# ndming/GS-2M

Measured on AMD Instinct MI355X. Metric: train views/s (fwd+bwd raster) at 1M Gaussians 1080p, higher is better.
Workload: dtype f32; 1 GPU; BASELINE configs[2] (c3): 1000000 synthetic Gaussians (SH deg 3), 1 camera 1920x1080 per GPU, feature_count=9, fwd+bwd at the op boundary; gaussians=1000000, visible=844909, num_rendered=2709460, width=1920, height=1080, feature_count=9, parallelism=view-parallel x1, views_per_rank=1

## Files before the change

gs-2m_amd/csrc/api.hip:

```cpp
#include "common.h"
#include <atomic>
#include <mutex>
#include <chrono>
#include <dlfcn.h>

#define HIP_TRY(expr)                          \
    do {                                       \
        hipError_t e_ = (expr);                \
        if (e_ != hipSuccess) return GS2M_ERR_HIP; \
    } while (0)

namespace {

uint32_t higher_msb(uint32_t n) {
    uint32_t msb = sizeof(n) * 4;
    uint32_t step = msb;
    while (step > 1) {
        step /= 2;
        if (n >> msb) msb += step; else msb -= step;
    }
    if (n >> msb) msb++;
    return msb;
}

// ... 6 lines not shown
};
LandRing g_land[64];
std::mutex g_land_mutex;
thread_local uint64_t t_last_token = 0;
thread_local long long t_rows_hint = -1;
thread_local long long t_units_hint = -1, t_units_from_token = -1;

static_assert(GS2M_NUM_STAGES == 10, "stage table");
enum Stage { ST_PREPROCESS = 0, ST_UNUSED1, ST_SCAN, ST_EMIT, ST_TILE_SORT, ST_LISTS, ST_BLEND_FWD, ST_UNUSED7,
             ST_BLEND_BWD, ST_GAUSSIAN_BWD, ST_COUNT };
constexpr int kMaxRecords = 8192;
struct Prof {
    std::atomic<int> mode{0};
    int n = 0;
    hipEvent_t ev[kMaxRecords][2];
    int stage[kMaxRecords];
    int created = 0;
    int every = 1;
    int seen3 = 0;
};
Prof g_prof;
std::mutex g_prof_mutex;
std::atomic<int> g_reference_binning{0};
std::atomic<int> g_spin_wait{1};
std::atomic<int> g_debug{0};
std::atomic<int> g_markers{0};

const char* const kStageNames[ST_COUNT] = {"preprocess", "-", "scan", "emit", "tile_sort", "depth_order+quad_lists", "blend_fwd", "-", "blend_bwd", "gaussian_bwd"};

struct Roctx {
    int (*push)(const char*) = nullptr;
    int (*pop)() = nullptr;
    bool tried = false;
    void load() {
        if (tried) return;
        tried = true;
        void* h = dlopen("libroctx64.so", RTLD_NOW | RTLD_GLOBAL);
        if (!h) h = dlopen("libroctx64.so.4", RTLD_NOW | RTLD_GLOBAL);
        if (!h) return;
        push = (int (*)(const char*))dlsym(h, "roctxRangePushA");
        pop = (int (*)())dlsym(h, "roctxRangePop");
    }
};
Roctx g_roctx;

struct StageTimer {
// ... 18 lines not shown
                (void)hipEventCreate(&g_prof.ev[slot][0]);
                (void)hipEventCreate(&g_prof.ev[slot][1]);
                g_prof.created = slot + 1;
            }
            g_prof.stage[slot] = stage;
        }
        (void)hipEventRecord(g_prof.ev[slot][0], s);
    }
    ~StageTimer() {
        if (slot >= 0) (void)hipEventRecord(g_prof.ev[slot][1], s);
        if (failed && g_debug.load(std::memory_order_relaxed) && *failed == 0) {
            hipError_t e = hipGetLastError();
            if (e == hipSuccess) e = hipStreamSynchronize(s);
            if (e != hipSuccess) *failed = stage + 1;
        }
        if (marked && g_roctx.pop) g_roctx.pop();
    }
};
#define DEBUG_CHECK()                                        \
    do {                                                     \
        if (failed_stage) return GS2M_ERR_STAGE(failed_stage - 1); \
    } while (0)

}

extern "C" {

char* gs2m_prealloc_alloc(size_t bytes, void* user) {
    gs2m_prealloc* p = static_cast<gs2m_prealloc*>(user);
    if (!p) return nullptr;
    p->requested = bytes;
    if (p->ptr && bytes <= p->capacity) return p->ptr;
    p->used_fallback = 1;
    return p->fallback ? p->fallback(bytes, p->fallback_user) : nullptr;
}

const char* gs2m_version(void) { return "gs2m_raster 0.5 (gfx950, round 5)"; }

static int forward_impl(gs2m_alloc_fn geometry_alloc, void* geometry_user, gs2m_alloc_fn binning_alloc,
                        void* binning_user, gs2m_alloc_fn image_alloc, void* image_user, int P, int D, int M,
                        const float* background, int width, int height, const float* means3D, const float* shs, const float* shs_rest,
                        const float* colors_precomp, const float* opacities, const float* scales, float scale_modifier,
                        const float* rotations, const float* cov3D_precomp, const float* features,
                        const float* viewmatrix, const float* projmatrix, const float* cam_pos, float tan_fovx,
                        float tan_fovy, int prefiltered, int feature_count, float* out_color, int* out_radii,
                        int* out_observe, float* out_buffer, void* stream_) {
// ... 262 lines not shown
    if (!sh_dc || !sh_rest) return GS2M_ERR_INVALID_ARG;
    return backward_impl(P, D, M, R, background, width, height, means3D, sh_dc, sh_rest, colors_precomp, scales, scale_modifier, rotations, cov3D_precomp, features, viewmatrix, projmatrix, campos, tan_fovx, tan_fovy, radii, buffer, geom_buffer, binning_buffer, image_buffer, feature_count, grad_colors, grad_buffer, dL_dmeans2D, dL_dconics, dL_dopacities, dL_dcolors, dL_dmeans3D, dL_dcov3D, dL_dsh_dc, dL_dsh_rest, dL_dscales, dL_drots, dL_dfeatures, scratch_alloc, scratch_user, stream_);
}

int gs2m_raster_mark_visible(int P, const float* means3D, const float* viewmatrix, const float* projmatrix,
                             uint8_t* present, void* stream_) {
    (void)projmatrix;
    if (P < 0) return GS2M_ERR_INVALID_ARG;
    if (P == 0) return GS2M_OK;
    if (!means3D || !viewmatrix || !present) return GS2M_ERR_INVALID_ARG;
    gs2m_launch_mark_visible(P, means3D, viewmatrix, present, (hipStream_t)stream_);
    HIP_TRY(hipGetLastError());
    return GS2M_OK;
}

int gs2m_set_reference_binning(int on) {
    g_reference_binning = on ? 1 : 0;
    return GS2M_OK;
}

int gs2m_set_tile_sort_policy(int policy) {
    if (policy < 0 || policy > 3) return GS2M_ERR_INVALID_ARG;
    gs2m_set_tile_sort_policy_impl(policy);
    return GS2M_OK;
}

int gs2m_set_debug(int on) {
    g_debug = on ? 1 : 0;
    return GS2M_OK;
}

int gs2m_set_markers(int on) {
    g_markers = on ? 1 : 0;
    if (on) {
        g_roctx.load();
        if (!g_roctx.push || !g_roctx.pop) return GS2M_ERR_UNSUPPORTED;
    }
    return GS2M_OK;
}

const char* gs2m_stage_name(int stage) { return stage >= 0 && stage < ST_COUNT ? kStageNames[stage] : "?"; }

int gs2m_set_spin_wait(int on) {
    g_spin_wait = on ? 1 : 0;
    return GS2M_OK;
}
// ... 119 lines not shown
```

gs-2m_amd/csrc/blend_bwd_q.hip:

```cpp
#include "common.h"

namespace {

typedef float v4f __attribute__((ext_vector_type(4)));
#ifdef GS2M_ROW_SECTORS
#define GS2M_ROW_ROUND(nv) ((((nv) + 7) / 8) * 8)
#else
#define GS2M_ROW_ROUND(nv) ((((nv) + 3) / 4) * 4)
#endif
typedef float v2f __attribute__((ext_vector_type(2)));
#ifndef GS2M_BWDQ_WAVES
#define GS2M_BWDQ_WAVES
#endif
#ifndef GS2M_BWDQ_UNROLL_B
#define GS2M_BWDQ_UNROLL_B 1
#endif

__device__ __forceinline__ void row_scan_affine2(float& Ax, float& Ay, float& Bx, float& By) {
#define GS2M_AFFINE_LEVEL(D)                                                             \
        "v_fmac_f32_dpp %2, %2, %0 row_shr:" #D " row_mask:0xf bank_mask:0xf\n\t"          \
        "v_fmac_f32_dpp %3, %3, %1 row_shr:" #D " row_mask:0xf bank_mask:0xf\n\t"          \
        "v_mul_f32_dpp %0, %0, %0 row_shr:" #D " row_mask:0xf bank_mask:0xf\n\t"           \
        "v_mul_f32_dpp %1, %1, %1 row_shr:" #D " row_mask:0xf bank_mask:0xf\n\t"
    asm("s_nop 1\n\t"
        GS2M_AFFINE_LEVEL(1)
        GS2M_AFFINE_LEVEL(2)
        GS2M_AFFINE_LEVEL(4)
        GS2M_AFFINE_LEVEL(8)
        : "+v"(Ax), "+v"(Ay), "+v"(Bx), "+v"(By));
#undef GS2M_AFFINE_LEVEL
}
__device__ __forceinline__ float row_shr1(float first, float v) {
    return __int_as_float(__builtin_amdgcn_update_dpp(__float_as_int(first), __float_as_int(v), 0x111 , 0xF, 0xF, false));
}

template <int FC>
__global__ void __launch_bounds__(64) GS2M_BWDQ_WAVES blend_bwd_q_kernel(
    const uint2* __restrict__ ranges, const uint2* __restrict__ qlist, const uint32_t* __restrict__ qlast,
    const uint32_t* __restrict__ qcount, const uint32_t* __restrict__ qrow,
    const float4* __restrict__ rec, int W, int H, int tiles_x, int tiles, const float* __restrict__ bg, int fc,
    const float* __restrict__ final_T,
    const uint32_t* __restrict__ n_contrib, const float* __restrict__ grad_color,
    const float* __restrict__ grad_buffer, float* __restrict__ rows) {
    constexpr int NV = ROW_FEAT + FC;
    constexpr int ROWF = GS2M_ROW_ROUND(NV);
    constexpr int RSTRIDE = ROWF;
    constexpr int NC = 3 + FC;
    constexpr int KK = (NC + 3) / 4;
#ifndef GS2M_BWDQ_GSTRIDE
#define GS2M_BWDQ_GSTRIDE 20
#endif
    constexpr int GST = GS2M_BWDQ_GSTRIDE;
    __shared__ __align__(16) float s_g[64][GST];
    __shared__ float2 s_T2[32];
    __shared__ float2 s_B2[32];
    __shared__ uint2 s_N2[32];
    __shared__ __align__(16) float s_out[16][ROWF];
    __shared__ uint32_t s_rowg[16];

    const int b = blockIdx.x;
    const int tile = (b >> 5) * 8 + (b & 7);
    const int quad = (b >> 3) & 3;
    if (tile >= tiles) return;
    const int lane = threadIdx.x;
    const int tile_x = tile % tiles_x, tile_y = tile / tiles_x;
    const int qx0 = tile_x * GS2M_TILE + (quad & 1) * 8, qy0 = tile_y * GS2M_TILE + (quad >> 1) * 8;
    if (qx0 >= W || qy0 >= H) return;
    const uint2 range = ranges[tile];

    uint32_t lastp;
    {
        const int px = qx0 + (lane & 7), py = qy0 + (lane >> 3);
        const bool inside = px < W && py < H;
        const size_t HW = (size_t)H * W, pix = (size_t)py * W + px;
        const float Tf = inside ? final_T[pix] : 0.f;
        lastp = inside ? n_contrib[pix] : 0u;
        float g[16];
#pragma unroll
        for (int k = 0; k < 16; k++) g[k] = 0.f;
        if (inside) {
            g[0] = grad_color[pix]; g[1] = grad_color[HW + pix]; g[2] = grad_color[2 * HW + pix];
#pragma unroll
            for (int ch = 0; ch < FC; ch++) g[3 + ch] = ch < fc ? grad_buffer[ch * HW + pix] : 0.f;
        }
#pragma unroll
        for (int q = 0; q < 4; q++)
            *reinterpret_cast<float4*>(&s_g[lane][4 * q]) = make_float4(g[4 * q], g[4 * q + 1], g[4 * q + 2], g[4 * q + 3]);
        const int pe = ((lane >> 3) * 4 + (lane & 3)) * 2 + ((lane >> 2) & 1);
        reinterpret_cast<float*>(s_T2)[pe] = Tf;
        reinterpret_cast<float*>(s_B2)[pe] = bg[0] * g[0] + bg[1] * g[1] + bg[2] * g[2];
        reinterpret_cast<uint32_t*>(s_N2)[pe] = lastp;
    }
    gs2m_sync();

    const int j = lane & 15, r = lane >> 4;
    const float qxr = (float)(qx0 + r), qyf = (float)qy0;
    const float halfW = 0.5f * W, halfH = 0.5f * H;

    float sx = 0.f, sy = 0.f, sA = 0.f, sB = 0.f, sC = 0.f, so = 0.f;
    float scB[KK];
#pragma unroll
    for (int k = 0; k < KK; k++) scB[k] = 0.f;
    const float* gA = &s_g[4 * (j & 3) + (j >> 2)][r];
    uint32_t spos = 0xFFFFFFFFu;
    const v2f pxf2 = {qxr, qxr + 4.0f};

    const uint32_t len = range.y - range.x;
    const uint2* list = qlist + (size_t)4 * range.x + (size_t)quad * len;
    const uint32_t* lrow = qrow + (size_t)4 * range.x + (size_t)quad * len;
    const int np = (int)qlast[tile * 4 + quad];
    const int ngroups = (np + 15) >> 4;
    struct Fill {
        float4 g0;
        float2 g1;
        float ch[KK];
        uint32_t pos1;
        uint32_t row;
    };
    struct Entry {
        uint2 e;
        uint32_t row;
    };
    auto load_entry = [&](int g) {
        const int p = np - 1 - (16 * g + j);
        Entry en;
        en.e = list[max(p, 0)];
        en.row = lrow[max(p, 0)];
        en.e.y = p >= 0 ? en.e.y + 1u : 0xFFFFFFFFu;
        return en;
    };
    auto load_fill = [&](const Entry en) {
        Fill f;
        const float4* p = rec + (size_t)(en.e.x & GS2M_GID_MASK) * REC_Q;
        f.g0 = p[REC_GEO0];
        f.g1 = *reinterpret_cast<const float2*>(p + REC_GEO1);
#pragma unroll
        for (int k = 0; k < KK; k++) f.ch[k] = reinterpret_cast<const float*>(p + REC_CH + k)[r];
        f.pos1 = en.e.y;
        f.row = en.row;
        return f;
    };
    auto row_ptr = [&](uint32_t row) -> float* {
        return reinterpret_cast<float*>(reinterpret_cast<float4*>(rows) + (size_t)(row * (uint32_t)(RSTRIDE / 4)));
    };
    Fill f;
    uint32_t row_cur = 0;
    Entry e_next = {make_uint2(0u, 0u), 0u};
    int g_cur = 0;
    auto issue_next = [&]() {
        if (g_cur + 1 < ngroups) f = load_fill(e_next);
        if (g_cur + 2 < ngroups) e_next = load_entry(g_cur + 2);
    };
    int pending = 0;
    auto flush_rows = [&]() {
        constexpr int RQ = ROWF / 4;
#pragma unroll
        for (int t0 = 0; t0 < 16 * RQ; t0 += GS2M_WAVE) {
            const int t = t0 + lane, e = t / RQ, q = t - e * RQ;
            if (t < 16 * RQ && e < pending)
                reinterpret_cast<float4*>(row_ptr(s_rowg[e]))[q] = *reinterpret_cast<const float4*>(&s_out[e][4 * q]);
        }
        pending = 0;
    };
    auto process_group = [&](int nvalid) {
        v4f acc1 = {0.f, 0.f, 0.f, 0.f};
        float U1 = 0.f, U2 = 0.f;
        v2f m0 = {0.f, 0.f}, m1 = {0.f, 0.f}, m2 = {0.f, 0.f};
        auto gc_block = [&](int b) {
            v4f a = {0.f, 0.f, 0.f, 0.f};
#pragma unroll
            for (int k = 0; k < KK; k++) a = __builtin_amdgcn_mfma_f32_16x16x4f32(gA[(16 * b) * GST + 4 * k], scB[k], a, 0, 0, 0);
            return a;
        };
        v4f gnext = gc_block(0);
// ... 82 lines not shown
            const auto x = __builtin_amdgcn_permlane32_swap(__float_as_uint(va), __float_as_uint(vb), false, false);
            const float hab = __uint_as_float(x[0]) + __uint_as_float(x[1]);
            const auto y = __builtin_amdgcn_permlane32_swap(__float_as_uint(vc), __float_as_uint(vd), false, false);
            const float hcd = __uint_as_float(y[0]) + __uint_as_float(y[1]);
            const auto z = __builtin_amdgcn_permlane16_swap(__float_as_uint(hab), __float_as_uint(hcd), false, false);
            return __uint_as_float(z[0]) + __uint_as_float(z[1]);
        };
        const v2f dxc = sx2 - pxf2;
        const float M0 = m0.x + m0.y, Sx = dxc.x * m0.x + dxc.y * m0.y, Sy = m1.x + m1.y;
        const float Sxx = (dxc.x * dxc.x) * m0.x + (dxc.y * dxc.y) * m0.y, Sxy = dxc.x * m1.x + dxc.y * m1.y, Syy = m2.x + m2.y;
        const float o0 = -halfW * (sA * Sx + sB * Sy), o1 = -halfH * (sC * Sy + sB * Sx), o2 = halfW * U1, o3 = halfH * U2;
        const float o7 = so > 0.f ? M0 * __builtin_amdgcn_rcpf(so) : 0.f;
        const float R1 = reduce4(o0, o2, o1, o3);
        const float R2 = reduce4(-0.5f * Sxx, -0.5f * Syy, -0.5f * Sxy, o7);
        s_out[j][r] = R1;
        s_out[j][4 + r] = R2;
        if (r == 0) s_rowg[j] = row_cur;
#pragma unroll
        for (int rr = 0; rr < 4; rr++)
            if (j < ROWF - ROW_COL) s_out[4 * r + rr][ROW_COL + j] = j < NC ? acc1[rr] : 0.f;
        pending = nvalid;
    };

    {
        const int n = (int)qcount[tile * 4 + quad];
        for (int i = np + lane; i < n; i += GS2M_WAVE) {
            float4* o4 = reinterpret_cast<float4*>(row_ptr(lrow[i]));
#pragma unroll
            for (int q4 = 0; q4 < ROWF / 4; q4++) o4[q4] = make_float4(0.f, 0.f, 0.f, 0.f);
        }
    }
    if (ngroups > 0) {
        f = load_fill(load_entry(0));
        e_next = load_entry(1);
        for (g_cur = 0; g_cur < ngroups; g_cur++) {
            sx = f.g0.x; sy = f.g0.y; sA = f.g0.z; sB = f.g0.w; sC = f.g1.x; so = f.g1.y;
#pragma unroll
            for (int k = 0; k < KK; k++) scB[k] = f.ch[k];
            spos = f.pos1;
            row_cur = f.row;
            process_group(min(16, np - 16 * g_cur));
        }
        asm volatile("s_waitcnt lgkmcnt(0)" ::: "memory");
        flush_rows();
    }
}

int fc_template(int fc) { return fc <= 1 ? 1 : (fc <= 5 ? 5 : (fc <= 9 ? 9 : 10)); }

}

int gs2m_row_floats(int fc) { return GS2M_ROW_ROUND(ROW_FEAT + fc_template(fc)); }

void gs2m_launch_blend_bwd_q(int W, int H, int tiles_x, int tiles_y, int fc, const float* bg, const GeomState& g,
                             const BinningState& b, const ImageState& im, const float* grad_color,
                             const float* grad_buffer, float* rows, hipStream_t s) {
    const int tiles = tiles_x * tiles_y;
    const int grid = ((tiles + 7) / 8) * 32;
#define GS2M_BWDQ(FC)                                                                                                      \
    blend_bwd_q_kernel<FC><<<grid, 64, 0, s>>>(im.ranges, b.qlist, im.qlast, im.qcount, b.qrow, g.rec, W, H, tiles_x, tiles, bg, fc, im.final_T, \
                                                  im.n_contrib, grad_color, grad_buffer, rows)
    switch (fc_template(fc)) {
        case 1: GS2M_BWDQ(1); break;
        case 5: GS2M_BWDQ(5); break;
        case 9: GS2M_BWDQ(9); break;
        default: GS2M_BWDQ(10); break;
    }
#undef GS2M_BWDQ
}
```

gs-2m_amd/csrc/blend_fwd_q.hip:

```cpp
#include "common.h"

namespace {

typedef float v2f __attribute__((ext_vector_type(2)));

template <int FC>
__global__ void __launch_bounds__(64) blend_fwd_q_kernel(
    const uint2* __restrict__ ranges, const uint2* __restrict__ qlist, const uint32_t* __restrict__ qcount,
    const float4* __restrict__ rec, int W, int H, int tiles_x, int tiles, const float* __restrict__ bg, int fc,
    float* __restrict__ out_color, float* __restrict__ out_buffer, float* __restrict__ final_T,
    uint32_t* __restrict__ n_contrib, int* __restrict__ observe, uint32_t* __restrict__ qlast) {
    constexpr int NC = 3 + FC;
    constexpr int KQ = (NC + 3) / 4;
    constexpr int NP = (NC + 1) / 2;

    const int b = blockIdx.x;
    const int tile = (b >> 5) * 8 + (b & 7);
    const int quad = (b >> 3) & 3;
    if (tile >= tiles) return;
    const int lane = threadIdx.x;
    const int tile_x = tile % tiles_x, tile_y = tile / tiles_x;
    const int qx0 = tile_x * GS2M_TILE + (quad & 1) * 8, qy0 = tile_y * GS2M_TILE + (quad >> 1) * 8;
    if (qx0 >= W || qy0 >= H) return;
    const int px = qx0 + (lane & 7), py = qy0 + (lane >> 3);
    const bool inside = px < W && py < H;
    const float pxf = (float)px, pyf = (float)py;

    const uint2 range = ranges[tile];
    const uint32_t len = range.y - range.x;
    const int n = __builtin_amdgcn_readfirstlane((int)qcount[tile * 4 + quad]);
    const uint2* list = qlist + (size_t)4 * range.x + (size_t)quad * len;

    constexpr int CH = 16;
    constexpr int NS = 2 + KQ;
    constexpr int BUFQ = NS * CH + CH / 2;
    __shared__ float4 s_buf[2 * BUFQ];
    uint32_t lds_zero;
    asm volatile("v_mov_b32 %0, 0" : "=v"(lds_zero));
    float4* const s_base = s_buf + lds_zero;
    auto q_at = [&](int buf, int slot, int jj) -> float4& { return s_base[buf * BUFQ + slot * CH + jj]; };
    auto e_at = [&](int buf, int jj) -> uint2& { return reinterpret_cast<uint2*>(s_base + buf * BUFQ + NS * CH)[jj]; };
    const int ej = lane & 15, eq = lane >> 4;
    auto quad_of = [](int slot) { return slot < 2 ? slot : slot + 1; };

    float T = 1.0f;
    uint32_t last_contributor = 0;
    v2f acc[NP];
#pragma unroll
    for (int k = 0; k < NP; k++) acc[k] = v2f{0.f, 0.f};
    typedef unsigned long long mask_t;
    mask_t live = __builtin_amdgcn_ballot_w64(inside);
    bool watch = true;
    int ilast = 0;

    auto eval = [&](const int i, const int buf, const int jj) {
        const float4 a = q_at(buf, 0, jj);
        const float2 b = *reinterpret_cast<const float2*>(&q_at(buf, 1, jj));
        float4 c[KQ];
#pragma unroll
        for (int q = 0; q < KQ; q++) c[q] = q_at(buf, 2 + q, jj);
        const uint2 ec = e_at(buf, jj);
        const float dx = a.x - pxf, dy = a.y - pyf;
        const float p2 = gs2m_power(dx, dy, a.z, a.w, b.x);
        const float alpha = fminf(0.99f, b.y * gs2m_exp(p2));
        const float test_T = T * (1.0f - alpha);
        const mask_t cand = live & __builtin_amdgcn_ballot_w64(p2 <= 0.0f) & __builtin_amdgcn_ballot_w64(alpha >= 1.0f / 255.0f);
        const mask_t fin = cand & __builtin_amdgcn_ballot_w64(test_T < 0.0001f);
        const mask_t contrib = cand & ~fin;
        live &= ~fin;
        if (contrib != 0ull) ilast = i + 1;
        float tw;
        asm("v_cndmask_b32_e64 %0, 0, %1, %2" : "=v"(tw) : "v"(T), "s"(contrib));
        const float w = alpha * tw;
        const v2f ww = {w, w};
#pragma unroll
        for (int q = 0; q < KQ; q++) {
            if (4 * q < NC) acc[2 * q] = __builtin_elementwise_fma(v2f{c[q].x, c[q].y}, ww, acc[2 * q]);
            if (4 * q + 2 < NC) acc[2 * q + 1] = __builtin_elementwise_fma(v2f{c[q].z, c[q].w}, ww, acc[2 * q + 1]);
        }
        const uint32_t pos1 = ec.y;
        asm("v_cndmask_b32_e64 %0, %0, %1, %2" : "+v"(last_contributor) : "v"(pos1), "s"(contrib));
        if (watch) {
            const mask_t half = contrib & __builtin_amdgcn_ballot_w64(T > 0.5f);
            if (half != 0ull) {
                if (lane == 0) atomicAdd(&observe[__builtin_amdgcn_readfirstlane(ec.x)], (int)__popcll(half));
            }
            watch = (live & __builtin_amdgcn_ballot_w64(T > 0.5f)) != 0ull;
        }
        asm("v_cndmask_b32_e64 %0, %0, %1, %2" : "+v"(T) : "v"(test_T), "s"(contrib));
        return live == 0ull;
    };

    const int nchunks = (n + CH - 1) / CH;
    auto load_entry = [&](int c) {
        return list[min(c * CH + ej, n - 1)];
    };
    struct Stage { float4 a, b; };
    auto load_quads = [&](const uint2 e) {
        Stage st;
        const float4* p = rec + (size_t)(e.x & GS2M_GID_MASK) * REC_Q;
        st.a = p[quad_of(eq)];
        st.b = eq + 4 < NS ? p[quad_of(eq + 4)] : make_float4(0.f, 0.f, 0.f, 0.f);
        return st;
    };
    auto park = [&](int buf, const uint2 e, const Stage& st) {
        q_at(buf, eq, ej) = st.a;
        if (eq + 4 < NS) q_at(buf, eq + 4, ej) = st.b;
        if (eq == 0) e_at(buf, ej) = make_uint2(e.x & GS2M_GID_MASK, e.y + 1u);
    };
    if (nchunks > 0) {
        uint2 e1 = load_entry(0);
        park(0, e1, load_quads(e1));
        e1 = nchunks > 1 ? load_entry(1) : e1;
        bool stop = false;
        for (int c = 0; c < nchunks && !stop; c++) {
            Stage st;
            const uint2 ecur = e1;
            if (c + 1 < nchunks) st = load_quads(ecur);
            if (c + 2 < nchunks) e1 = load_entry(c + 2);
            const int base = c * CH, buf = c & 1;
#pragma unroll
            for (int jj = 0; jj < CH; jj++) {
                if (base + jj >= n) break;
                if (eval(base + jj, buf, jj)) { stop = true; break; }
            }
            if (c + 1 < nchunks && !stop) park(buf ^ 1, ecur, st);
        }
    }

    if (lane == 0) qlast[tile * 4 + quad] = (uint32_t)ilast;
    if (inside) {
        const size_t HW = (size_t)H * W;
        const size_t pix = (size_t)py * W + px;
        final_T[pix] = T;
        n_contrib[pix] = last_contributor;
        out_color[pix] = acc[0][0] + T * bg[0];
        out_color[HW + pix] = acc[0][1] + T * bg[1];
        out_color[2 * HW + pix] = acc[1][0] + T * bg[2];
#pragma unroll
        for (int ch = 0; ch < GS2M_NUM_FEATURES; ch++) {
            const int cch = 3 + ch;
            out_buffer[ch * HW + pix] = (ch < FC && ch < fc) ? acc[(cch >> 1) < NP ? (cch >> 1) : 0][cch & 1] : 0.0f;
        }
    }
}

}

void gs2m_launch_blend_fwd_q(int W, int H, int tiles_x, int tiles_y, int fc, const float* bg, const GeomState& g,
                             const BinningState& b, const ImageState& im, float* out_color, float* out_buffer,
                             int* out_observe, hipStream_t s) {
    const int tiles = tiles_x * tiles_y;
    const int grid = ((tiles + 7) / 8) * 32;
    const int fct = fc <= 1 ? 1 : (fc <= 5 ? 5 : (fc <= 9 ? 9 : 10));
#define GS2M_FWDQ(FC)                                                                                                   \
    blend_fwd_q_kernel<FC><<<grid, 64, 0, s>>>(im.ranges, b.qlist, im.qcount, g.rec, W, H, tiles_x, tiles, bg, fc, out_color, \
                                               out_buffer, im.final_T, im.n_contrib, out_observe, im.qlast)
    switch (fct) {
        case 1: GS2M_FWDQ(1); break;
        case 5: GS2M_FWDQ(5); break;
        case 9: GS2M_FWDQ(9); break;
        default: GS2M_FWDQ(10); break;
    }
#undef GS2M_FWDQ
}
```

gs-2m_amd/csrc/common.h:

```cpp
#pragma once
#include <hip/hip_runtime.h>
#include <stdint.h>
#include <stddef.h>
#include "../../include/gs2m_raster.h"

typedef float gs2m_v4f __attribute__((ext_vector_type(4)));
template <typename T> __device__ __forceinline__ T gs2m_ldnt(const T* p) { return __builtin_nontemporal_load(p); }
__device__ __forceinline__ float4 gs2m_ldnt(const float4* p) {
    const gs2m_v4f t = __builtin_nontemporal_load(reinterpret_cast<const gs2m_v4f*>(p));
    return make_float4(t.x, t.y, t.z, t.w);
}
template <typename T> __device__ __forceinline__ void gs2m_stnt(T* p, T v) { __builtin_nontemporal_store(v, p); }
__device__ __forceinline__ void gs2m_stnt(float4* p, float4 v) {
    const gs2m_v4f t = {v.x, v.y, v.z, v.w};
    __builtin_nontemporal_store(t, reinterpret_cast<gs2m_v4f*>(p));
}

#define GS2M_ALIGN 256
#define GS2M_WAVE 64

#define REC_Q 8
#define REC_GEO0 0
#define REC_GEO1 1
#define REC_BIN 2
// ... 162 lines not shown
#define GS2M_LAND_HUNITS 1
#define GS2M_LAND_PREFILTERED 2
#define GS2M_LAND_ROWS 3
#define GS2M_CNT_ROWS 2
#define GS2M_CNT_HUNITS 3
#define GS2M_CNT_SPAN_MID 4
#define GS2M_CNT_SPAN_LONG 5

void gs2m_launch_preprocess(int P, int D, int M, const float* means3D, const float* scales, float scale_modifier,
                            const float* rotations, const float* opacities, const float* shs, const float* shs_rest,
                            const float* cov3D_precomp, const float* colors_precomp, const float* features,
                            const float* viewmatrix, const float* projmatrix, const float* cam_pos, int W, int H,
                            float tan_fovx, float tan_fovy, float focal_x, float focal_y, int tiles_x, int tiles_y,
                            int* radii, int* observe_zero, const GeomState& g, int shrink, const ZeroJobs& zero, hipStream_t s);
void gs2m_launch_blockscan(int P, const GeomState& g, uint32_t* landing, hipStream_t s);
void gs2m_launch_emit(int P, int W, int H, int tiles_x, int tile_bits, const GeomState& g, const BinningState& b, uint32_t heavy_units,
                      uint32_t crowded, uint32_t* landing, const ZeroJobs& zero, hipStream_t s);
void gs2m_launch_recount_heavy(int P, const GeomState& g, hipStream_t s);
void gs2m_launch_heavy_reduce(float* rows, int rowf, const BinningState& b, const GeomState& g, long long heavy_units, hipStream_t s);
void gs2m_set_tile_sort_policy_impl(int policy);
void gs2m_launch_tile_sort(size_t tiles, int tiles_x, int tiles_y, size_t R, const BinningState& b, const ImageState& im, const GeomState& g, hipStream_t s);
hipError_t gs2m_zero_async(void* p, size_t bytes, hipStream_t s);

void gs2m_launch_blend_fwd_q(int W, int H, int tiles_x, int tiles_y, int fc, const float* bg, const GeomState& g,
                             const BinningState& b, const ImageState& im, float* out_color, float* out_buffer,
                             int* out_observe, hipStream_t s);
void gs2m_launch_blend_bwd_q(int W, int H, int tiles_x, int tiles_y, int fc, const float* bg, const GeomState& g,
                             const BinningState& b, const ImageState& im, const float* grad_color,
                             const float* grad_buffer, float* rows, hipStream_t s);
int gs2m_row_floats(int fc);
void gs2m_launch_gaussian_bwd(int P, int D, int M, const float* means3D, const float* shs, const float* shs_rest,
                              const float* colors_precomp,
                              const float* scales, float scale_modifier, const float* rotations,
                              const float* cov3D_precomp, const float* viewmatrix, const float* projmatrix,
                              const float* campos, int W, int H, float tan_fovx, float tan_fovy, const int* radii,
                              int fc, const GeomState& g, const float* rows, int rowf, bool have_rows,
                              float* dL_dmeans2D, float* dL_dconics, float* dL_dopacities, float* dL_dcolors,
                              float* dL_dmeans3D, float* dL_dcov3D, float* dL_dshs, float* dL_dshs_rest, float* dL_dscales,
                              float* dL_drots, float* dL_dfeatures, hipStream_t s);
void gs2m_launch_prefiltered_check(int P, const float* means3D, const float* viewmatrix, uint32_t* flag, hipStream_t s);
void gs2m_launch_mark_visible(int P, const float* means3D, const float* viewmatrix, uint8_t* present, hipStream_t s);

#ifdef __HIPCC__
__device__ __forceinline__ float u2f(uint32_t u) { return __uint_as_float(u); }
__device__ __forceinline__ uint32_t f2u(float f) { return __float_as_uint(f); }

// ... 100 lines not shown
```

gs-2m_amd/gs2m_native.py:

```python
import ctypes as C
import os
import subprocess

_HERE = os.path.dirname(os.path.abspath(__file__))
CSRC = os.path.join(_HERE, "csrc")
LIB_PATH = os.environ.get("GS2M_LIB", os.path.join(CSRC, "libgs2m_raster.so"))

ALLOC_FN = C.CFUNCTYPE(C.c_void_p, C.c_size_t, C.c_void_p)


class Prealloc(C.Structure):
    _fields_ = [("ptr", C.c_void_p), ("capacity", C.c_size_t), ("fallback", ALLOC_FN), ("fallback_user", C.c_void_p),
                ("used_fallback", C.c_int), ("requested", C.c_size_t)]


class Layout(C.Structure):
    _fields_ = [(n, C.c_uint64) for n in (
        "geom_bytes", "rec", "tiles_touched", "depth_key", "rect", "gauss_rows", "clamped", "wave_rowbase", "counters",
        "binning_bytes", "point_list", "tile_keys", "qlist", "qrow",
        "image_bytes", "final_T", "n_contrib", "ranges", "qcount")]


class STREAM(C.c_void_p):
    """`void* stream` as an entry point's LAST parameter: the function enqueues GPU work (call it through `launch`)."""
# ... 5 lines not shown
                                p, p, p, s]),
    "gs2m_raster_backward": (i, [i, i, i, i, p, i, i, p, p, p, p, f, p, p, p, p, p, p, f, f, p, p, p, p, p, i, p, p, p,
                                 p, p, p, p, p, p, p, p, p, A, p, s]),
    "gs2m_raster_mark_visible": (i, [i, p, p, p, p, s]),
    "gs2m_knn_dist2": (i, [i, p, p, A, p, s]),
    "gs2m_debug_layout": (i, [i, i, i, i, C.POINTER(Layout)]),
    "gs2m_set_reference_binning": (i, [i]),
    "gs2m_raster_forward_split_sh": (i, [A, p, A, p, A, p, i, i, i, p, i, i, p, p, p, p, p, p, f, p, p, p, p, p, p, f,
                                         f, i, i, p, p, p, p, s]),
    "gs2m_raster_backward_split_sh": (i, [i, i, i, i, p, i, i, p, p, p, p, p, f, p, p, p, p, p, p, f, f, p, p, p, p, p,
                                          i, p, p, p, p, p, p, p, p, p, p, p, p, p, A, p, s]),
    "gs2m_pack_features_forward": (i, [i, p, p, p, p, p, p, p, p, i, i, p, s]),
    "gs2m_pack_features_backward": (i, [i, p, p, p, p, p, i, i, p, p, p, p, p, p, s]),
    "gs2m_gbuffer_post_forward": (i, [i, i, p, p, p, i, p, p, p, s]),
    "gs2m_gbuffer_post_backward": (i, [i, i, p, p, p, i, p, p, p, s]),
    "gs2m_gbuffer_maps_backward": (i, [i, i, p, p, p, i, p, p, p, p, p, p, p, p, p, s]),
    "gs2m_sobel_normal_forward": (i, [i, i, p, p, p, p, f, f, f, f, p, s]),
    "gs2m_sobel_normal_backward": (i, [i, i, p, p, p, p, f, f, f, f, p, p, p, s]),
    "gs2m_activate_forward": (i, [i, p, p, p, p, p, p, p, p, p, p, p, p, s]),
    "gs2m_activate_backward": (i, [i, p, p, p, p, p, p, p, p, p, p, p, p, p, p, p, p, p, p, s]),
    "gs2m_set_spin_wait": (i, [i]),
    "gs2m_set_sort_tickets": (i, [i]),
    "gs2m_set_tile_sort_policy": (i, [i]),
    "gs2m_prealloc_alloc": (p, [C.c_size_t, p]),
    "gs2m_set_debug": (i, [i]),
    "gs2m_set_markers": (i, [i]),
    "gs2m_stage_name": (C.c_char_p, [i]),
    "gs2m_raster_forward_token": (ull, []),
    "gs2m_raster_dense_rows": (ll, [ull]),
    "gs2m_raster_backward_rows_hint": (i, [ll]),
    "gs2m_debug_tile_sort": (i, [i, p, p, p, p, p, p, p, p, p, p, s]),
    "gs2m_profile_mode": (i, [i]),
    "gs2m_profile_sampling": (i, [i]),
    "gs2m_profile_collect": (i, [C.POINTER(C.c_float), C.POINTER(C.c_int), i]),
    "gs2m_version": (C.c_char_p, []),
    "gs2m_texture_cube_forward": (i, [i, i, i, p, p, p, p, p, s]),
    "gs2m_texture_cube_backward": (i, [i, i, i, p, p, p, p, p, i, s]),
    "gs2m_texture_2d_clamp_forward": (i, [i, i, i, i, p, p, p, s]),
    "gs2m_texture_2d_clamp_backward": (i, [i, i, i, i, p, p, p, s]),
    "gs2m_diffuse_cubemap_forward": (i, [i, p, p, s]),
    "gs2m_diffuse_cubemap_backward": (i, [i, p, p, s]),
    "gs2m_cubemap_texel_table": (i, [i, p, s]),
    "gs2m_specular_cubemap_forward": (i, [i, f, f, p, p, p, s]),
    "gs2m_specular_cubemap_backward": (i, [i, f, f, p, p, p, s]),
    "gs2m_specular_cubemap_normalized_forward": (i, [i, f, f, p, p, p, p, s]),
    "gs2m_specular_cubemap_normalized_backward": (i, [i, f, f, p, p, p, p, p, s]),
# ... 154 lines not shown
    import torch
    if optional and (t is None or t.numel() == 0):
        return t
    if not isinstance(t, torch.Tensor) or not t.is_cuda:
        raise RuntimeError(f"{who}: `{name}` must be a CUDA tensor on a HIP device; there is no CPU path")
    if t.dtype != torch.float32:
        raise RuntimeError(f"{who}: `{name}` must be float32, got {t.dtype}")
    if shape is not None and tuple(t.shape) != tuple(shape):
        raise RuntimeError(f"{who}: `{name}` must have shape {tuple(shape)}, got {tuple(t.shape)}")
    return t.contiguous()


def set_debug(on):
    check(lib().gs2m_set_debug(int(bool(on))), "gs2m_set_debug")


def set_markers(on):
    check(lib().gs2m_set_markers(int(bool(on))), "gs2m_set_markers")


def reset_modes():
    L = lib()
    L.gs2m_set_reference_binning(0); L.gs2m_set_spin_wait(1); L.gs2m_set_debug(0); L.gs2m_set_sort_tickets(0); L.gs2m_set_tile_sort_policy(0)
    L.gs2m_set_markers(0); L.gs2m_profile_mode(0)


def debug_layout(P, R, W, H):
    lay = Layout()
    check(lib().gs2m_debug_layout(P, R, W, H, C.byref(lay)), "gs2m_debug_layout")
    return lay


def set_sort_tickets(on):
    check(lib().gs2m_set_sort_tickets(int(bool(on))), "gs2m_set_sort_tickets")


def set_tile_sort_policy(policy):
    check(lib().gs2m_set_tile_sort_policy(int(policy)), "gs2m_set_tile_sort_policy")


def set_spin_wait(on):
    check(lib().gs2m_set_spin_wait(int(bool(on))), "gs2m_set_spin_wait")


def profile_mode(mode, every=1):
    check(lib().gs2m_profile_sampling(int(every)), "gs2m_profile_sampling")
    check(lib().gs2m_profile_mode(int(mode)), "gs2m_profile_mode")


def profile_collect():
    n = len(STAGES)
    ms = (C.c_float * n)()
    cnt = (C.c_int * n)()
    check(lib().gs2m_profile_collect(ms, cnt, n), "gs2m_profile_collect")
    return {STAGES[k]: (float(ms[k]), int(cnt[k])) for k in range(n)}


def set_reference_binning(on):
    check(lib().gs2m_set_reference_binning(1 if on else 0), "gs2m_set_reference_binning")
```

include/gs2m_raster.h:

```cpp
#ifndef GS2M_RASTER_H
#define GS2M_RASTER_H

#include <stddef.h>
#include <stdint.h>

#ifdef __cplusplus
extern "C" {
#endif

#define GS2M_NUM_CHANNELS 3
#define GS2M_NUM_FEATURES 10
#define GS2M_TILE 16

#define GS2M_OK 0
#define GS2M_ERR_INVALID_ARG (-1)
#define GS2M_ERR_HIP (-2)
#define GS2M_ERR_ALLOC (-3)
#define GS2M_ERR_UNSUPPORTED (-4)
#define GS2M_ERR_PREFILTERED (-5)
#define GS2M_ERR_STAGE(st) (-100 - (st))

typedef char* (*gs2m_alloc_fn)(size_t bytes, void* user);

int gs2m_raster_forward(
// ... 132 lines not shown
                               const float* dL_droughness, const float* dL_dmetallic, float* dL_dbuffer, void* stream);

int gs2m_sobel_normal_forward(int width, int height, const float* depth, const float* alpha, const float* bg,
                              const float* view, float fx, float fy, float cx, float cy, float* sobel_map, void* stream);
int gs2m_sobel_normal_backward(int width, int height, const float* depth, const float* alpha, const float* bg,
                               const float* view, float fx, float fy, float cx, float cy, const float* dL_dsobel,
                               float* dL_ddepth, float* dL_dalpha, void* stream);

int gs2m_activate_forward(int P, const float* scaling, const float* rotation, const float* opacity, const float* albedo,
                          const float* roughness, const float* metallic, float* scales, float* rotations, float* opacities,
                          float* albedo_a, float* roughness_a, float* metallic_a, void* stream);
int gs2m_activate_backward(int P, const float* rotation, const float* scales, const float* opacities, const float* albedo_a,
                           const float* roughness_a, const float* metallic_a, const float* dL_dscales,
                           const float* dL_drotations, const float* dL_dopacities, const float* dL_dalbedo_a,
                           const float* dL_droughness_a, const float* dL_dmetallic_a, float* dL_dscaling, float* dL_drotation,
                           float* dL_dopacity, float* dL_dalbedo, float* dL_droughness, float* dL_dmetallic, void* stream);

int gs2m_set_spin_wait(int on);

int gs2m_set_sort_tickets(int on);

int gs2m_set_tile_sort_policy(int policy);

typedef struct gs2m_prealloc {
    char* ptr;
    size_t capacity;
    gs2m_alloc_fn fallback;
    void* fallback_user;
    int used_fallback;
    size_t requested;
} gs2m_prealloc;
char* gs2m_prealloc_alloc(size_t bytes, void* user);

int gs2m_set_debug(int on);
int gs2m_set_markers(int on);
const char* gs2m_stage_name(int stage);


unsigned long long gs2m_raster_forward_token(void);
long long gs2m_raster_dense_rows(unsigned long long token);
int gs2m_raster_backward_rows_hint(long long dense_rows);

int gs2m_debug_tile_sort(int tiles, const unsigned* ranges_raw, unsigned* ranges, const unsigned* slot_sorted, const unsigned* e_rec,
                         const unsigned* wave_rowbase, unsigned* point_list, unsigned* row_tmp,
                         unsigned* qlist, unsigned* qrow, unsigned* qcount, void* stream);

// ... 12 lines not shown
```

Measured before the change: 857.1 views/s.

## Make blend fwd/bwd kernels persistent with cross-quadrant list prefetch

Converts the forward and backward quadrant blend kernels from one block per quadrant into a persistent grid. The grid is sized from occupancy times CU count, and each block strides over quadrant jobs. While the current quadrant is processed, each block prefetches the header and first list entries of its next quadrant, removing launch/ramp tail costs and the exposed latency at the start of each list. This adds an occupancy query on the host (cached per kernel and device), and the static job striding may load-balance worse than hardware block scheduling when per-quadrant work is uneven.

```diff
diff --git a/gs-2m_amd/csrc/api.hip b/gs-2m_amd/csrc/api.hip
--- a/gs-2m_amd/csrc/api.hip
+++ b/gs-2m_amd/csrc/api.hip
@@ -52,6 +52,7 @@
 Prof g_prof;
 std::mutex g_prof_mutex;
 std::atomic<int> g_reference_binning{0};
+std::atomic<int> g_blend_policy{1};
 std::atomic<int> g_spin_wait{1};
 std::atomic<int> g_debug{0};
 std::atomic<int> g_markers{0};
@@ -116,6 +117,32 @@
         if (failed_stage) return GS2M_ERR_STAGE(failed_stage - 1); \
     } while (0)
 
+}
+
+int gs2m_blend_grid(int jobs, const void* kernel) {
+    if (g_blend_policy.load() == 0) return jobs;
+    struct Known { const void* kernel; int device, waves; };
+    static std::mutex mutex;
+    static Known known[64];
+    static int count = 0;
+    int device = 0;
+    if (hipGetDevice(&device) != hipSuccess) return jobs;
+    int waves = 0;
+    {
+        std::lock_guard<std::mutex> lock(mutex);
+        for (int k = 0; k < count; k++)
+            if (known[k].kernel == kernel && known[k].device == device) waves = known[k].waves;
+    }
+    if (waves == 0) {
+        int per_cu = 0, cus = 0;
+        if (hipOccupancyMaxActiveBlocksPerMultiprocessor(&per_cu, kernel, GS2M_WAVE, 0) != hipSuccess ||
+            hipDeviceGetAttribute(&cus, hipDeviceAttributeMultiprocessorCount, device) != hipSuccess || per_cu <= 0 || cus <= 0)
+            return jobs;
+        waves = std::max(8, per_cu * cus / 8 * 8);
+        std::lock_guard<std::mutex> lock(mutex);
+        if (count < 64) known[count++] = {kernel, device, waves};
+    }
+    return std::min(jobs, waves);
 }
 
 extern "C" {
@@ -424,6 +451,12 @@
 int gs2m_set_tile_sort_policy(int policy) {
     if (policy < 0 || policy > 3) return GS2M_ERR_INVALID_ARG;
     gs2m_set_tile_sort_policy_impl(policy);
+    return GS2M_OK;
+}
+
+int gs2m_set_blend_policy(int policy) {
+    if (policy < 0 || policy > 1) return GS2M_ERR_INVALID_ARG;
+    g_blend_policy = policy;
     return GS2M_OK;
 }
 
diff --git a/gs-2m_amd/csrc/blend_bwd_q.hip b/gs-2m_amd/csrc/blend_bwd_q.hip
--- a/gs-2m_amd/csrc/blend_bwd_q.hip
+++ b/gs-2m_amd/csrc/blend_bwd_q.hip
@@ -38,7 +38,7 @@
 __global__ void __launch_bounds__(64) GS2M_BWDQ_WAVES blend_bwd_q_kernel(
     const uint2* __restrict__ ranges, const uint2* __restrict__ qlist, const uint32_t* __restrict__ qlast,
     const uint32_t* __restrict__ qcount, const uint32_t* __restrict__ qrow,
-    const float4* __restrict__ rec, int W, int H, int tiles_x, int tiles, const float* __restrict__ bg, int fc,
+    const float4* __restrict__ rec, int W, int H, int tiles_x, int tiles, int njobs, const float* __restrict__ bg, int fc,
     const float* __restrict__ final_T,
     const uint32_t* __restrict__ n_contrib, const float* __restrict__ grad_color,
     const float* __restrict__ grad_buffer, float* __restrict__ rows) {
@@ -58,43 +58,71 @@
     __shared__ __align__(16) float s_out[16][ROWF];
     __shared__ uint32_t s_rowg[16];
 
-    const int b = blockIdx.x;
-    const int tile = (b >> 5) * 8 + (b & 7);
-    const int quad = (b >> 3) & 3;
-    if (tile >= tiles) return;
     const int lane = threadIdx.x;
-    const int tile_x = tile % tiles_x, tile_y = tile / tiles_x;
-    const int qx0 = tile_x * GS2M_TILE + (quad & 1) * 8, qy0 = tile_y * GS2M_TILE + (quad >> 1) * 8;
-    if (qx0 >= W || qy0 >= H) return;
-    const uint2 range = ranges[tile];
-
-    uint32_t lastp;
-    {
-        const int px = qx0 + (lane & 7), py = qy0 + (lane >> 3);
+    const int stride = gridDim.x;
+    struct Quadrant { int tile, quad, qx0, qy0; bool valid; };
+    auto decode = [&](long long jb) {
+        Quadrant q;
+        q.tile = (int)(jb >> 5) * 8 + (int)(jb & 7);
+        q.quad = (int)(jb >> 3) & 3;
+        const int tile_x = q.tile % tiles_x, tile_y = q.tile / tiles_x;
+        q.qx0 = tile_x * GS2M_TILE + (q.quad & 1) * 8, q.qy0 = tile_y * GS2M_TILE + (q.quad >> 1) * 8;
+        q.valid = jb < njobs && q.tile < tiles && q.qx0 < W && q.qy0 < H;
+        return q;
+    };
+    struct Head { uint2 range; uint32_t np, n; };
+    auto fetch_head = [&](long long jb) {
+        Head h = {make_uint2(0u, 0u), 0u, 0u};
+        const Quadrant q = decode(jb);
+        if (q.valid) {
+            h.range = ranges[q.tile];
+            h.np = qlast[q.tile * 4 + q.quad];
+            h.n = qcount[q.tile * 4 + q.quad];
+        }
+        return h;
+    };
+    auto list_offset = [&](const Head& h, int quad) {
+        const uint32_t lo = __builtin_amdgcn_readfirstlane(h.range.x), hi = __builtin_amdgcn_readfirstlane(h.range.y);
+        return (size_t)4 * lo + (size_t)quad * (hi - lo);
+    };
+
+    struct Pix {
+        float Tf;
+        uint32_t lastp;
+        float g[NC];
+    };
+    auto load_pix = [&](const Quadrant& q) {
+        Pix p;
+        const int px = q.qx0 + (lane & 7), py = q.qy0 + (lane >> 3);
         const bool inside = px < W && py < H;
         const size_t HW = (size_t)H * W, pix = (size_t)py * W + px;
-        const float Tf = inside ? final_T[pix] : 0.f;
-        lastp = inside ? n_contrib[pix] : 0u;
+        p.Tf = inside ? final_T[pix] : 0.f;
+        p.lastp = inside ? n_contrib[pix] : 0u;
+#pragma unroll
+        for (int k = 0; k < NC; k++) p.g[k] = 0.f;
+        if (inside) {
+            p.g[0] = grad_color[pix]; p.g[1] = grad_color[HW + pix]; p.g[2] = grad_color[2 * HW + pix];
+#pragma unroll
+            for (int ch = 0; ch < FC; ch++) p.g[3 + ch] = ch < fc ? grad_buffer[ch * HW + pix] : 0.f;
+        }
+        return p;
+    };
+    auto store_pix = [&](const Pix& p) {
         float g[16];
 #pragma unroll
-        for (int k = 0; k < 16; k++) g[k] = 0.f;
-        if (inside) {
-            g[0] = grad_color[pix]; g[1] = grad_color[HW + pix]; g[2] = grad_color[2 * HW + pix];
-#pragma unroll
-            for (int ch = 0; ch < FC; ch++) g[3 + ch] = ch < fc ? grad_buffer[ch * HW + pix] : 0.f;
-        }
+        for (int k = 0; k < 16; k++) g[k] = k < NC ? p.g[k < NC ? k : 0] : 0.f;
 #pragma unroll
         for (int q = 0; q < 4; q++)
             *reinterpret_cast<float4*>(&s_g[lane][4 * q]) = make_float4(g[4 * q], g[4 * q + 1], g[4 * q + 2], g[4 * q + 3]);
         const int pe = ((lane >> 3) * 4 + (lane & 3)) * 2 + ((lane >> 2) & 1);
-        reinterpret_cast<float*>(s_T2)[pe] = Tf;
+        reinterpret_cast<float*>(s_T2)[pe] = p.Tf;
         reinterpret_cast<float*>(s_B2)[pe] = bg[0] * g[0] + bg[1] * g[1] + bg[2] * g[2];
-        reinterpret_cast<uint32_t*>(s_N2)[pe] = lastp;
-    }
-    gs2m_sync();
+        reinterpret_cast<uint32_t*>(s_N2)[pe] = p.lastp;
+    };
 
     const int j = lane & 15, r = lane >> 4;
-    const float qxr = (float)(qx0 + r), qyf = (float)qy0;
+    float qyf = 0.f;
+    v2f pxf2 = {0.f, 0.f};
     const float halfW = 0.5f * W, halfH = 0.5f * H;
 
     float sx = 0.f, sy = 0.f, sA = 0.f, sB = 0.f, sC = 0.f, so = 0.f;
@@ -103,13 +131,11 @@
     for (int k = 0; k < KK; k++) scB[k] = 0.f;
     const float* gA = &s_g[4 * (j & 3) + (j >> 2)][r];
     uint32_t spos = 0xFFFFFFFFu;
-    const v2f pxf2 = {qxr, qxr + 4.0f};
-
-    const uint32_t len = range.y - range.x;
-    const uint2* list = qlist + (size_t)4 * range.x + (size_t)quad * len;
-    const uint32_t* lrow = qrow + (size_t)4 * range.x + (size_t)quad * len;
-    const int np = (int)qlast[tile * 4 + quad];
-    const int ngroups = (np + 15) >> 4;
+
+    const uint2 *list = qlist, *listN = qlist;
+    const uint32_t *lrow = qrow, *lrowN = qrow;
+    int np = 0, npN = 0;
+    int ngroups = 0, total = 0;
     struct Fill {
         float4 g0;
         float2 g1;
@@ -122,10 +148,11 @@
         uint32_t row;
     };
     auto load_entry = [&](int g) {
-        const int p = np - 1 - (16 * g + j);
+        const bool cur = g < ngroups;
+        const int p = cur ? np - 1 - (16 * g + j) : npN - 1 - (16 * (g - ngroups) + j);
         Entry en;
-        en.e = list[max(p, 0)];
-        en.row = lrow[max(p, 0)];
+        en.e = (cur ? list : listN)[max(p, 0)];
+        en.row = (cur ? lrow : lrowN)[max(p, 0)];
         en.e.y = p >= 0 ? en.e.y + 1u : 0xFFFFFFFFu;
         return en;
     };
@@ -147,9 +174,10 @@
     uint32_t row_cur = 0;
     Entry e_next = {make_uint2(0u, 0u), 0u};
     int g_cur = 0;
+    Quadrant qN = decode(0);
     auto issue_next = [&]() {
-        if (g_cur + 1 < ngroups) f = load_fill(e_next);
-        if (g_cur + 2 < ngroups) e_next = load_entry(g_cur + 2);
+        if (g_cur + 1 < total) f = load_fill(e_next);
+        if (g_cur + 2 < total) e_next = load_entry(g_cur + 2);
     };
     int pending = 0;
     auto flush_rows = [&]() {
@@ -278,27 +306,60 @@
         pending = nvalid;
     };
 
-    {
-        const int n = (int)qcount[tile * 4 + quad];
+    bool have_fill = false;
+    bool have_e = false;
+    Head h0 = fetch_head(blockIdx.x), h1 = fetch_head((long long)blockIdx.x + stride);
+    for (long long jb = blockIdx.x; jb < njobs; jb += stride) {
+        const Head h2 = fetch_head(jb + 2ll * stride);
+        const Quadrant q = decode(jb);
+        qN = decode(jb + stride);
+        np = __builtin_amdgcn_readfirstlane((int)h0.np);
+        const int n = __builtin_amdgcn_readfirstlane((int)h0.n);
+#ifdef GS2M_BLEND_NO_PREFETCH
+        npN = 0;
+#else
+        npN = __builtin_amdgcn_readfirstlane((int)h1.np);
+#endif
+        {
+            const size_t o = list_offset(h0, q.quad), oN = list_offset(h1, qN.quad);
+            list = qlist + o; lrow = qrow + o;
+            listN = qlist + oN; lrowN = qrow + oN;
+        }
+        h0 = h1;
+        h1 = h2;
+        if (!q.valid) continue;
+        ngroups = (np + 15) >> 4;
+        total = ngroups + ((npN + 15) >> 4);
+        qyf = (float)q.qy0;
+        pxf2 = v2f{(float)(q.qx0 + r), (float)(q.qx0 + r) + 4.0f};
+
         for (int i = np + lane; i < n; i += GS2M_WAVE) {
             float4* o4 = reinterpret_cast<float4*>(row_ptr(lrow[i]));
 #pragma unroll
             for (int q4 = 0; q4 < ROWF / 4; q4++) o4[q4] = make_float4(0.f, 0.f, 0.f, 0.f);
         }
-    }
-    if (ngroups > 0) {
-        f = load_fill(load_entry(0));
-        e_next = load_entry(1);
-        for (g_cur = 0; g_cur < ngroups; g_cur++) {
-            sx = f.g0.x; sy = f.g0.y; sA = f.g0.z; sB = f.g0.w; sC = f.g1.x; so = f.g1.y;
-#pragma unroll
-            for (int k = 0; k < KK; k++) scB[k] = f.ch[k];
-            spos = f.pos1;
-            row_cur = f.row;
-            process_group(min(16, np - 16 * g_cur));
-        }
-        asm volatile("s_waitcnt lgkmcnt(0)" ::: "memory");
-        flush_rows();
+        if (ngroups > 0) {
+            const Pix pix = load_pix(q);
+            if (!have_fill) {
+                f = load_fill(load_entry(0));
+                have_e = false;
+            }
+            if (!have_e && total > 1) e_next = load_entry(1);
+            store_pix(pix);
+            gs2m_sync();
+            for (g_cur = 0; g_cur < ngroups; g_cur++) {
+                sx = f.g0.x; sy = f.g0.y; sA = f.g0.z; sB = f.g0.w; sC = f.g1.x; so = f.g1.y;
+#pragma unroll
+                for (int k = 0; k < KK; k++) scB[k] = f.ch[k];
+                spos = f.pos1;
+                row_cur = f.row;
+                process_group(min(16, np - 16 * g_cur));
+            }
+            have_fill = total > ngroups;
+            have_e = total > ngroups + 1;
+            asm volatile("s_waitcnt lgkmcnt(0)" ::: "memory");
+            flush_rows();
+        }
     }
 }
 
@@ -312,10 +373,11 @@
                              const BinningState& b, const ImageState& im, const float* grad_color,
                              const float* grad_buffer, float* rows, hipStream_t s) {
     const int tiles = tiles_x * tiles_y;
-    const int grid = ((tiles + 7) / 8) * 32;
+    const int njobs = ((tiles + 7) / 8) * 32;
 #define GS2M_BWDQ(FC)                                                                                                      \
-    blend_bwd_q_kernel<FC><<<grid, 64, 0, s>>>(im.ranges, b.qlist, im.qlast, im.qcount, b.qrow, g.rec, W, H, tiles_x, tiles, bg, fc, im.final_T, \
-                                                  im.n_contrib, grad_color, grad_buffer, rows)
+    blend_bwd_q_kernel<FC><<<gs2m_blend_grid(njobs, (const void*)blend_bwd_q_kernel<FC>), 64, 0, s>>>(                     \
+        im.ranges, b.qlist, im.qlast, im.qcount, b.qrow, g.rec, W, H, tiles_x, tiles, njobs, bg, fc, im.final_T,           \
+        im.n_contrib, grad_color, grad_buffer, rows)
     switch (fc_template(fc)) {
         case 1: GS2M_BWDQ(1); break;
         case 5: GS2M_BWDQ(5); break;
diff --git a/gs-2m_amd/csrc/blend_fwd_q.hip b/gs-2m_amd/csrc/blend_fwd_q.hip
--- a/gs-2m_amd/csrc/blend_fwd_q.hip
+++ b/gs-2m_amd/csrc/blend_fwd_q.hip
@@ -7,29 +7,39 @@
 template <int FC>
 __global__ void __launch_bounds__(64) blend_fwd_q_kernel(
     const uint2* __restrict__ ranges, const uint2* __restrict__ qlist, const uint32_t* __restrict__ qcount,
-    const float4* __restrict__ rec, int W, int H, int tiles_x, int tiles, const float* __restrict__ bg, int fc,
+    const float4* __restrict__ rec, int W, int H, int tiles_x, int tiles, int njobs, const float* __restrict__ bg, int fc,
     float* __restrict__ out_color, float* __restrict__ out_buffer, float* __restrict__ final_T,
     uint32_t* __restrict__ n_contrib, int* __restrict__ observe, uint32_t* __restrict__ qlast) {
     constexpr int NC = 3 + FC;
     constexpr int KQ = (NC + 3) / 4;
     constexpr int NP = (NC + 1) / 2;
 
-    const int b = blockIdx.x;
-    const int tile = (b >> 5) * 8 + (b & 7);
-    const int quad = (b >> 3) & 3;
-    if (tile >= tiles) return;
     const int lane = threadIdx.x;
-    const int tile_x = tile % tiles_x, tile_y = tile / tiles_x;
-    const int qx0 = tile_x * GS2M_TILE + (quad & 1) * 8, qy0 = tile_y * GS2M_TILE + (quad >> 1) * 8;
-    if (qx0 >= W || qy0 >= H) return;
-    const int px = qx0 + (lane & 7), py = qy0 + (lane >> 3);
-    const bool inside = px < W && py < H;
-    const float pxf = (float)px, pyf = (float)py;
-
-    const uint2 range = ranges[tile];
-    const uint32_t len = range.y - range.x;
-    const int n = __builtin_amdgcn_readfirstlane((int)qcount[tile * 4 + quad]);
-    const uint2* list = qlist + (size_t)4 * range.x + (size_t)quad * len;
+    const int stride = gridDim.x;
+    struct Quadrant { int tile, quad, qx0, qy0; bool valid; };
+    auto decode = [&](long long jb) {
+        Quadrant q;
+        q.tile = (int)(jb >> 5) * 8 + (int)(jb & 7);
+        q.quad = (int)(jb >> 3) & 3;
+        const int tile_x = q.tile % tiles_x, tile_y = q.tile / tiles_x;
+        q.qx0 = tile_x * GS2M_TILE + (q.quad & 1) * 8, q.qy0 = tile_y * GS2M_TILE + (q.quad >> 1) * 8;
+        q.valid = jb < njobs && q.tile < tiles && q.qx0 < W && q.qy0 < H;
+        return q;
+    };
+    struct Head { uint2 range; uint32_t n; };
+    auto fetch_head = [&](long long jb) {
+        Head h = {make_uint2(0u, 0u), 0u};
+        const Quadrant q = decode(jb);
+        if (q.valid) {
+            h.range = ranges[q.tile];
+            h.n = qcount[q.tile * 4 + q.quad];
+        }
+        return h;
+    };
+    auto list_of = [&](const Head& h, int quad) {
+        const uint32_t lo = __builtin_amdgcn_readfirstlane(h.range.x), hi = __builtin_amdgcn_readfirstlane(h.range.y);
+        return qlist + (size_t)4 * lo + (size_t)quad * (hi - lo);
+    };
 
     constexpr int CH = 16;
     constexpr int NS = 2 + KQ;
@@ -43,13 +53,12 @@
     const int ej = lane & 15, eq = lane >> 4;
     auto quad_of = [](int slot) { return slot < 2 ? slot : slot + 1; };
 
+    float pxf = 0.f, pyf = 0.f;
     float T = 1.0f;
     uint32_t last_contributor = 0;
     v2f acc[NP];
-#pragma unroll
-    for (int k = 0; k < NP; k++) acc[k] = v2f{0.f, 0.f};
     typedef unsigned long long mask_t;
-    mask_t live = __builtin_amdgcn_ballot_w64(inside);
+    mask_t live = 0ull;
     bool watch = true;
     int ilast = 0;
 
@@ -91,10 +100,6 @@
         return live == 0ull;
     };
 
-    const int nchunks = (n + CH - 1) / CH;
-    auto load_entry = [&](int c) {
-        return list[min(c * CH + ej, n - 1)];
-    };
     struct Stage { float4 a, b; };
     auto load_quads = [&](const uint2 e) {
         Stage st;
@@ -108,39 +113,85 @@
         if (eq + 4 < NS) q_at(buf, eq + 4, ej) = st.b;
         if (eq == 0) e_at(buf, ej) = make_uint2(e.x & GS2M_GID_MASK, e.y + 1u);
     };
-    if (nchunks > 0) {
-        uint2 e1 = load_entry(0);
-        park(0, e1, load_quads(e1));
-        e1 = nchunks > 1 ? load_entry(1) : e1;
-        bool stop = false;
-        for (int c = 0; c < nchunks && !stop; c++) {
-            Stage st;
-            const uint2 ecur = e1;
-            if (c + 1 < nchunks) st = load_quads(ecur);
-            if (c + 2 < nchunks) e1 = load_entry(c + 2);
-            const int base = c * CH, buf = c & 1;
-#pragma unroll
-            for (int jj = 0; jj < CH; jj++) {
-                if (base + jj >= n) break;
-                if (eval(base + jj, buf, jj)) { stop = true; break; }
-            }
-            if (c + 1 < nchunks && !stop) park(buf ^ 1, ecur, st);
-        }
-    }
-
-    if (lane == 0) qlast[tile * 4 + quad] = (uint32_t)ilast;
-    if (inside) {
-        const size_t HW = (size_t)H * W;
-        const size_t pix = (size_t)py * W + px;
-        final_T[pix] = T;
-        n_contrib[pix] = last_contributor;
-        out_color[pix] = acc[0][0] + T * bg[0];
-        out_color[HW + pix] = acc[0][1] + T * bg[1];
-        out_color[2 * HW + pix] = acc[1][0] + T * bg[2];
-#pragma unroll
-        for (int ch = 0; ch < GS2M_NUM_FEATURES; ch++) {
-            const int cch = 3 + ch;
-            out_buffer[ch * HW + pix] = (ch < FC && ch < fc) ? acc[(cch >> 1) < NP ? (cch >> 1) : 0][cch & 1] : 0.0f;
+
+    int buf = 0;
+    bool parked = false;
+    bool have_e1 = false;
+    uint2 e1 = make_uint2(0u, 0u);
+    Head h0 = fetch_head(blockIdx.x), h1 = fetch_head((long long)blockIdx.x + stride);
+    for (long long b = blockIdx.x; b < njobs; b += stride) {
+        const Head h2 = fetch_head(b + 2ll * stride);
+        const Quadrant q = decode(b), qN = decode(b + stride);
+        const int n = __builtin_amdgcn_readfirstlane((int)h0.n);
+#ifdef GS2M_BLEND_NO_PREFETCH
+        const int nN = 0;
+#else
+        const int nN = __builtin_amdgcn_readfirstlane((int)h1.n);
+#endif
+        const uint2* list = list_of(h0, q.quad);
+        const uint2* listN = list_of(h1, qN.quad);
+        h0 = h1;
+        h1 = h2;
+        if (!q.valid) continue;
+        const int px = q.qx0 + (lane & 7), py = q.qy0 + (lane >> 3);
+        const bool inside = px < W && py < H;
+        pxf = (float)px, pyf = (float)py;
+        T = 1.0f;
+        last_contributor = 0;
+#pragma unroll
+        for (int k = 0; k < NP; k++) acc[k] = v2f{0.f, 0.f};
+        live = __builtin_amdgcn_ballot_w64(inside);
+        watch = true;
+        ilast = 0;
+
+        const int nchunks = (n + CH - 1) / CH, total = nchunks + (nN + CH - 1) / CH;
+        auto load_entry = [&](int k) {
+            const bool cur = k < nchunks;
+            const uint2* l = cur ? list : listN;
+            const int kk = cur ? k : k - nchunks, nn = cur ? n : nN;
+            return l[min(kk * CH + ej, nn - 1)];
+        };
+        if (nchunks > 0) {
+            if (!parked) {
+                const uint2 e0 = load_entry(0);
+                park(buf, e0, load_quads(e0));
+                have_e1 = false;
+            }
+            if (!have_e1 && total > 1) e1 = load_entry(1);
+            bool stop = false;
+            int c = 0;
+            for (; c < nchunks && !stop; c++) {
+                Stage st;
+                const uint2 ecur = e1;
+                if (c + 1 < total) st = load_quads(ecur);
+                if (c + 2 < total) e1 = load_entry(c + 2);
+                const int base = c * CH;
+#pragma unroll
+                for (int jj = 0; jj < CH; jj++) {
+                    if (base + jj >= n) break;
+                    if (eval(base + jj, buf, jj)) { stop = true; break; }
+                }
+                if (c + 1 < total && (!stop || c + 1 >= nchunks)) park(buf ^ 1, ecur, st);
+                buf ^= 1;
+            }
+            parked = c == nchunks && total > nchunks;
+            have_e1 = c == nchunks && total > nchunks + 1;
+        }
+
+        if (lane == 0) qlast[q.tile * 4 + q.quad] = (uint32_t)ilast;
+        if (inside) {
+            const size_t HW = (size_t)H * W;
+            const size_t pix = (size_t)py * W + px;
+            final_T[pix] = T;
+            n_contrib[pix] = last_contributor;
+            out_color[pix] = acc[0][0] + T * bg[0];
+            out_color[HW + pix] = acc[0][1] + T * bg[1];
+            out_color[2 * HW + pix] = acc[1][0] + T * bg[2];
+#pragma unroll
+            for (int ch = 0; ch < GS2M_NUM_FEATURES; ch++) {
+                const int cch = 3 + ch;
+                out_buffer[ch * HW + pix] = (ch < FC && ch < fc) ? acc[(cch >> 1) < NP ? (cch >> 1) : 0][cch & 1] : 0.0f;
+            }
         }
     }
 }
@@ -151,11 +202,12 @@
                              const BinningState& b, const ImageState& im, float* out_color, float* out_buffer,
                              int* out_observe, hipStream_t s) {
     const int tiles = tiles_x * tiles_y;
-    const int grid = ((tiles + 7) / 8) * 32;
+    const int njobs = ((tiles + 7) / 8) * 32;
     const int fct = fc <= 1 ? 1 : (fc <= 5 ? 5 : (fc <= 9 ? 9 : 10));
 #define GS2M_FWDQ(FC)                                                                                                   \
-    blend_fwd_q_kernel<FC><<<grid, 64, 0, s>>>(im.ranges, b.qlist, im.qcount, g.rec, W, H, tiles_x, tiles, bg, fc, out_color, \
-                                               out_buffer, im.final_T, im.n_contrib, out_observe, im.qlast)
+    blend_fwd_q_kernel<FC><<<gs2m_blend_grid(njobs, (const void*)blend_fwd_q_kernel<FC>), 64, 0, s>>>(                  \
+        im.ranges, b.qlist, im.qcount, g.rec, W, H, tiles_x, tiles, njobs, bg, fc, out_color, out_buffer, im.final_T,   \
+        im.n_contrib, out_observe, im.qlast)
     switch (fct) {
         case 1: GS2M_FWDQ(1); break;
         case 5: GS2M_FWDQ(5); break;
diff --git a/gs-2m_amd/csrc/common.h b/gs-2m_amd/csrc/common.h
--- a/gs-2m_amd/csrc/common.h
+++ b/gs-2m_amd/csrc/common.h
@@ -208,6 +208,7 @@
 void gs2m_launch_tile_sort(size_t tiles, int tiles_x, int tiles_y, size_t R, const BinningState& b, const ImageState& im, const GeomState& g, hipStream_t s);
 hipError_t gs2m_zero_async(void* p, size_t bytes, hipStream_t s);
 
+int gs2m_blend_grid(int jobs, const void* kernel);
 void gs2m_launch_blend_fwd_q(int W, int H, int tiles_x, int tiles_y, int fc, const float* bg, const GeomState& g,
                              const BinningState& b, const ImageState& im, float* out_color, float* out_buffer,
                              int* out_observe, hipStream_t s);
diff --git a/gs-2m_amd/gs2m_native.py b/gs-2m_amd/gs2m_native.py
--- a/gs-2m_amd/gs2m_native.py
+++ b/gs-2m_amd/gs2m_native.py
@@ -51,6 +51,7 @@
     "gs2m_set_spin_wait": (i, [i]),
     "gs2m_set_sort_tickets": (i, [i]),
     "gs2m_set_tile_sort_policy": (i, [i]),
+    "gs2m_set_blend_policy": (i, [i]),
     "gs2m_prealloc_alloc": (p, [C.c_size_t, p]),
     "gs2m_set_debug": (i, [i]),
     "gs2m_set_markers": (i, [i]),
@@ -251,6 +252,7 @@
 def reset_modes():
     L = lib()
     L.gs2m_set_reference_binning(0); L.gs2m_set_spin_wait(1); L.gs2m_set_debug(0); L.gs2m_set_sort_tickets(0); L.gs2m_set_tile_sort_policy(0)
+    L.gs2m_set_blend_policy(1)
     L.gs2m_set_markers(0); L.gs2m_profile_mode(0)
 
 
@@ -266,6 +268,10 @@
 
 def set_tile_sort_policy(policy):
     check(lib().gs2m_set_tile_sort_policy(int(policy)), "gs2m_set_tile_sort_policy")
+
+
+def set_blend_policy(policy):
+    check(lib().gs2m_set_blend_policy(int(policy)), "gs2m_set_blend_policy")
 
 
 def set_spin_wait(on):
diff --git a/include/gs2m_raster.h b/include/gs2m_raster.h
--- a/include/gs2m_raster.h
+++ b/include/gs2m_raster.h
@@ -178,6 +178,8 @@
 
 int gs2m_set_tile_sort_policy(int policy);
 
+int gs2m_set_blend_policy(int policy);
+
 typedef struct gs2m_prealloc {
     char* ptr;
     size_t capacity;
```

New measurement: 759.6 views/s. 11.4% lower.
